# OpenResearchInstitute/opv-cxx-demod

Measured on AMD Instinct MI355X. Metric: IQ Msamples/s demod+Viterbi (×real-time @2.168MSPS); BER vs ref, higher is better.
Workload: dtype f64; 1 GPU; configs[3]: 64 concurrent IQ streams/GPU x 1000 frames, -s semantics, amp 2000, f0 -2000..+2000 Hz across the 64 streams of a shard (SURVEY.md §8d C4: edge streams on the AFC clamp, outside the +/-1530 Hz search span), Eb/N0 16 dB; streams_per_gpu=64, parallelism=streams sharded 64/GPU, no data-path collective

## Files before the change

### opv-cxx-demod_amd/csrc/k_sync_track.hip

```cpp
#include <hip/hip_runtime.h>
#include <math.h>
#include <stdint.h>

#include "opv_device.h"

namespace {

struct Corr { double raw, norm; };

__device__ inline Corr window_corr(const double* __restrict__ soft, uint32_t mask, uint64_t last) {
    const uint32_t w0 = (uint32_t)(last - (OPV_SYNC_BITS - 1));
    double sum = 0.0, energy = 0.0;
#pragma unroll
    for (int i = 0; i < OPV_SYNC_BITS; ++i) {
        const double s = soft[(w0 + (uint32_t)i) & mask];
        const double pat = ((OPV_SYNC_WORD >> (OPV_SYNC_BITS - 1 - i)) & 1u) ? -1.0 : 1.0;
        sum += s * pat;
        energy += fabs(s);
    }
    Corr c;
    c.raw = sum;
    c.norm = energy < 100.0 ? 0.0 : sum / energy;
    return c;
}

}

extern "C" __global__ __launch_bounds__(64) void k_sync_track(OpvStream* __restrict__ streams) {
    OpvStream& st = streams[blockIdx.x];
    const int lane = threadIdx.x;
    const double* __restrict__ soft = st.soft;
    const uint32_t mask = (uint32_t)(st.cap_soft - 1);
    const uint64_t n = st.n_soft;

    int state = st.trk_state, collecting = st.trk_collecting, misses = st.trk_misses;
    uint64_t anchor = st.trk_anchor, next = st.trk_next;
    double quality = st.trk_quality;
    uint32_t n_frames = st.n_frames, n_events = st.n_events;
    int overflow = st.overflow;
    if (lane == 0) st.dec_from = n_frames;

    auto event = [&](int kind, int count, uint64_t sym, double corr, double raw) {
        if (lane == 0) {
            OpvEventRec& e = st.events[n_events % st.cap_events];
            e.kind = kind; e.count = count; e.sym_idx = sym; e.corr = corr; e.raw = raw;
        }
        ++n_events;
    };
    int sync_ok = st.trk_sync_ok, stalled = 0;
    auto frames_full = [&]() { return n_frames - st.frames_popped >= st.cap_frames; };
    auto release = [&](uint64_t at) {
        if (lane == 0) {
            OpvFrameRec& f = st.frec[n_frames % st.cap_frames];
            f.payload_sym = anchor + 1;
            f.release_sym = at;
            f.quality = quality;
            f.sync_ok = sync_ok;
            f.pad = 0;
            st.metrics[n_frames % st.cap_frames] = INT32_MIN;
        }
        ++n_frames;
        collecting = 0;
    };

    for (;;) {
        if (overflow) break;
        if (state == 0) {
            uint64_t pos = next < (OPV_SYNC_BITS - 1) ? (uint64_t)(OPV_SYNC_BITS - 1) : next;
            bool found = false;
            while (pos < n) {
                const uint64_t cand = pos + (uint64_t)lane;
                Corr c = {0.0, 0.0};
                bool ok = false;
                if (cand < n) {
                    c = window_corr(soft, mask, cand);
                    ok = (c.raw >= 5000.0) && (c.norm >= 0.85);
                }
                const unsigned long long m = __ballot(ok);
                if (m) {
                    const int first = __ffsll((long long)m) - 1;
                    const uint64_t s = pos + (uint64_t)first;
                    const double nrm = __shfl(c.norm, first, 64), raw = __shfl(c.raw, first, 64);
                    state = 1;
                    sync_ok = 1;
                    quality = nrm;
                    anchor = s;
                    collecting = 1;
                    event(1, 0, s, nrm, raw);
                    next = s + 1;
                    found = true;
                    break;
                }
                pos += 64;
            }
            if (!found) { next = n; break; }
        } else if (state == 1) {
            const uint64_t r = anchor + OPV_CODED;
            if (r >= n) break;
            if (frames_full()) { stalled = 2; break; }
            release(r);
            state = 2;
            misses = 0;
            event(2, (int)n_frames, r, 0.0, 0.0);
            next = r + 1;
        } else {
            if (collecting) {
                const uint64_t r = anchor + OPV_CODED;
                if (r >= n) break;
                if (frames_full()) { stalled = 2; break; }
                release(r);
                next = r + 1;
                continue;
            }
            const uint64_t c = anchor + OPV_FSYMS;
            if (c >= n) break;
            const Corr k = window_corr(soft, mask, c);
            next = c + 1;
            if (k.norm >= 0.70) {
                misses = 0;
                quality = k.norm;
                collecting = 1;
                sync_ok = 1;
                event(3, 0, c, k.norm, k.raw);
            } else {
                ++misses;
                event(4, misses, c, k.norm, k.raw);
                if (misses >= 5) {
                    state = 0;
                    collecting = 0;
                    event(5, 0, c, k.norm, k.raw);
                    continue;
                }
                quality = k.norm;
                collecting = 1;
                sync_ok = 0;
            }
            anchor = c;
        }
    }

    if (lane == 0) {
        st.trk_state = state; st.trk_collecting = collecting; st.trk_misses = misses;
        st.trk_anchor = anchor; st.trk_next = next; st.trk_quality = quality;
        st.n_frames = n_frames; st.n_events = n_events; st.trk_sync_ok = sync_ok;
        st.stalled |= stalled;
    }
}
```

Baseline: 9306 Msamples/s.

## Batch tracked-state sync checks across wavefront lanes per iteration

```diff
diff --git a/opv-cxx-demod_amd/csrc/k_sync_track.hip b/opv-cxx-demod_amd/csrc/k_sync_track.hip
--- a/opv-cxx-demod_amd/csrc/k_sync_track.hip
+++ b/opv-cxx-demod_amd/csrc/k_sync_track.hip
@@ -47,6 +47,7 @@
         }
         ++n_events;
     };
+    const int width = st.cap_events > 64u ? 64 : (int)st.cap_events - 1;
     int sync_ok = st.trk_sync_ok, stalled = 0;
     auto frames_full = [&]() { return n_frames - st.frames_popped >= st.cap_frames; };
     auto release = [&](uint64_t at) {
@@ -114,6 +115,65 @@
             }
             const uint64_t c = anchor + OPV_FSYMS;
             if (c >= n) break;
+            if (width >= 2 && c + OPV_FSYMS < n) {
+                const uint64_t cl = anchor + (uint64_t)OPV_FSYMS * (uint64_t)(lane + 1);
+                const bool valid = lane < width && cl < n;
+                Corr k = {0.0, 0.0};
+                if (valid) k = window_corr(soft, mask, cl);
+                const bool hit = valid && k.norm >= 0.70;
+                const uint32_t held = n_frames - st.frames_popped;
+                const uint32_t room = held >= st.cap_frames ? 0u : st.cap_frames - held;
+                const bool rel_ok = valid && cl + OPV_CODED < n && (uint32_t)lane < room;
+                const unsigned long long mv = __ballot(valid), mh = __ballot(hit), mr = __ballot(rel_ok);
+                const unsigned long long hits_to_here = mh & ((2ull << lane) - 1ull);
+                const int run = hits_to_here ? lane - (63 - __clzll((long long)hits_to_here)) : lane + 1 + misses;
+                const unsigned long long mf = __ballot(valid && !hit && run >= 5);
+                const int n_valid = __popcll(mv), n_rel = __popcll(mr);
+                const int reach = n_valid < n_rel + 1 ? n_valid : n_rel + 1;
+                const int fifth = mf ? __ffsll((long long)mf) - 1 : 64;
+                const bool lost = fifth < reach;
+                const int n_chk = lost ? fifth + 1 : reach;
+                const int n_out = lost ? fifth : (n_rel < n_chk ? n_rel : n_chk);
+                __syncthreads();
+                if (lane < n_chk) {
+                    OpvEventRec& e = st.events[(n_events + (uint32_t)lane) % st.cap_events];
+                    e.kind = hit ? 3 : 4; e.count = hit ? 0 : run; e.sym_idx = cl; e.corr = k.norm; e.raw = k.raw;
+                    if (lost && lane == fifth) {
+                        OpvEventRec& l = st.events[(n_events + (uint32_t)n_chk) % st.cap_events];
+                        l.kind = 5; l.count = 0; l.sym_idx = cl; l.corr = k.norm; l.raw = k.raw;
+                    }
+                }
+                if (lane < n_out) {
+                    const uint32_t slot = (n_frames + (uint32_t)lane) % st.cap_frames;
+                    OpvFrameRec& f = st.frec[slot];
+                    f.payload_sym = cl + 1;
+                    f.release_sym = cl + OPV_CODED;
+                    f.quality = k.norm;
+                    f.sync_ok = hit ? 1 : 0;
+                    f.pad = 0;
+                    st.metrics[slot] = INT32_MIN;
+                }
+                __syncthreads();
+                const int last = lost ? n_chk - 2 : n_chk - 1;
+                const uint64_t c_end = anchor + (uint64_t)OPV_FSYMS * (uint64_t)n_chk;
+                misses = __shfl(hit ? 0 : run, n_chk - 1, 64);
+                if (last >= 0) {
+                    quality = __shfl(k.norm, last, 64);
+                    sync_ok = (int)((mh >> last) & 1ull);
+                    anchor += (uint64_t)OPV_FSYMS * (uint64_t)(last + 1);
+                }
+                n_events += (uint32_t)n_chk + (lost ? 1u : 0u);
+                n_frames += (uint32_t)n_out;
+                if (lost) {
+                    state = 0;
+                    collecting = 0;
+                    next = c_end + 1;
+                } else {
+                    collecting = n_out < n_chk;
+                    next = (collecting ? c_end : c_end + OPV_CODED) + 1;
+                }
+                continue;
+            }
             const Corr k = window_corr(soft, mask, c);
             next = c + 1;
             if (k.norm >= 0.70) {
```

Result: no change. 9320 Msamples/s, median of 6 (+0.2%).
